# ymxlzgy/commonscenes

Measured on AMD Instinct MI355X. Metric: DDIM denoise steps/sec (32 objects, 16^3 latent), higher is better.
Workload: dtype f32 (operands as fp16 hi+lo pairs, fp32 accumulate)

## Files before the change

### commonscenes_amd/csrc/cs_epilogue.h

```cpp
#pragma once
#include "cs_common.h"

typedef unsigned cs_u32x4 __attribute__((ext_vector_type(4)));

template <class D, class M>
__device__ __forceinline__ f32x4 cs_epi_terms4(const D& d, f32x4 v, M m, int n) {
  if (d.bias) v += *reinterpret_cast<const f32x4*>(d.bias + n);
  if (d.scale) v = v * *reinterpret_cast<const f32x4*>(d.scale + n) + *reinterpret_cast<const f32x4*>(d.shift + n);
  if (d.rowvec) v += *reinterpret_cast<const f32x4*>(d.rowvec + (int64_t)(m / d.rv_rows) * d.ldrv + n);
  if (d.act != CS_ACT_NONE) {
#pragma unroll
    for (int e = 0; e < 4; ++e) v[e] = cs_act(v[e], d.act);
  }
  if (d.res) v += *reinterpret_cast<const f32x4*>(d.res + (int64_t)m * d.ldr + n);
  return v;
}
template <class D>
__device__ __forceinline__ float cs_epi_terms1(const D& d, float v, float bias, float scale, float shift, int m, int n) {
  v += bias;
  if (d.scale) v = v * scale + shift;
  if (d.rowvec) v += d.rowvec[(int64_t)(m / d.rv_rows) * d.ldrv + n];
  v = cs_act(v, d.act);
  if (d.res) v += d.res[(int64_t)m * d.ldr + n];
  return v;
}

__device__ __forceinline__ f32x4 cs_geglu4(f32x4 x, const f32x4& g) {
#pragma unroll
  for (int e = 0; e < 4; ++e) x[e] = x[e] * cs_gelu(g[e]);
  return x;
}

__device__ __forceinline__ cs_u32x4 cs_pair16(const f32x4& v, float out_scale, bool odd, float& oamax) {
  typedef _Float16 h4 __attribute__((ext_vector_type(4)));
  typedef unsigned u32x2 __attribute__((ext_vector_type(2)));
  h4 hi, lo;
#pragma unroll
  for (int e = 0; e < 4; ++e) {
    const float o = v[e] * out_scale;
    oamax = fmaxf(oamax, fabsf(o));
    hi[e] = (_Float16)o;
    lo[e] = (_Float16)(o - (float)hi[e]);
  }
  const u32x2 H = __builtin_bit_cast(u32x2, hi), L = __builtin_bit_cast(u32x2, lo);
  const u32x2 send = odd ? H : L;
  u32x2 recv;
  recv[0] = (unsigned)__builtin_amdgcn_update_dpp(0, (int)send[0], 0xB1, 0xF, 0xF, true);
  recv[1] = (unsigned)__builtin_amdgcn_update_dpp(0, (int)send[1], 0xB1, 0xF, 0xF, true);
  cs_u32x4 r;
  r[0] = odd ? recv[0] : H[0];
  r[1] = odd ? recv[1] : H[1];
  r[2] = odd ? L[0] : recv[0];
  r[3] = odd ? L[1] : recv[1];
  return r;
}
__device__ __forceinline__ cs_u32x4 cs_pair16_half32(const f32x4& v, float out_scale, float& oamax) {
  typedef _Float16 h4 __attribute__((ext_vector_type(4)));
  typedef unsigned u32x2 __attribute__((ext_vector_type(2)));
  h4 hi, lo;
#pragma unroll
  for (int e = 0; e < 4; ++e) {
    const float o = v[e] * out_scale;
    oamax = fmaxf(oamax, fabsf(o));
    hi[e] = (_Float16)o;
    lo[e] = (_Float16)(o - (float)hi[e]);
  }
  const u32x2 H = __builtin_bit_cast(u32x2, hi), L = __builtin_bit_cast(u32x2, lo);
  const auto s0 = __builtin_amdgcn_permlane32_swap(H[0], L[0], false, false);
  const auto s1 = __builtin_amdgcn_permlane32_swap(H[1], L[1], false, false);
  cs_u32x4 r;
  r[0] = s0[0];
  r[1] = s1[0];
  r[2] = s0[1];
  r[3] = s1[1];
  return r;
}
__device__ __forceinline__ int cs_pair_off(int col) { return (col >> 4) * 64 + ((col & 8) ? 32 : 0) + ((col & 4) ? 16 : 0); }
template <class D>
__device__ __forceinline__ void cs_pair_flag(const D& d, bool opair, float oamax) {
  if (opair && d.status && oamax >= 65504.f) atomicOr(d.status, CS_STATUS_F16X3_OVERFLOW);
}

__device__ __forceinline__ void cs_colsum_lanes16(double (*sc)[64], const double (&x)[4], int rl, int cl, double (&tot)[4]) {
  __syncthreads();
#pragma unroll
  for (int e = 0; e < 4; ++e) sc[rl][cl * 4 + e] = x[e];
  __syncthreads();
  if (rl == 0) {
#pragma unroll
    for (int e = 0; e < 4; ++e) {
      double t = 0.0;
      for (int r2 = 0; r2 < 16; ++r2) t += sc[r2][cl * 4 + e];
      tot[e] = t;
    }
  }
}
template <class D>
__device__ __forceinline__ void cs_colsum_staged(const D& d, const float* col, int ld, int rows, int tile, int n) {
  double ts = 0.0, tq = 0.0;
  for (int r2 = 0; r2 < rows; ++r2) {
    const double x = (double)col[r2 * ld];
    ts += x;
    tq += x * x;
  }
  double* o = d.gn_part + ((int64_t)tile * d.gn_ld + n) * 2;
  o[0] = ts;
  o[1] = tq;
}
```

### commonscenes_amd/csrc/cs_gemm_f16x3.hip

```cpp
#include <cstdlib>
#include <cstring>
#include "cs_f16x3.h"
#include "cs_epilogue.h"
#include <type_traits>
#include <utility>

namespace {

using cs16::h8;
using cs16::split8;
using cs16::wait_vmcnt;
using cs16::BKH;
using cs16::A_SCALE_DEFAULT;
using cs16::OOB;
constexpr int MAX_TAPS = 27;
#ifndef CS_ABLATE
#define CS_ABLATE 0
#endif

struct CsClsBatch {
  const void* w[8];
  const void* w_lo[8];
  float acc_scale[8];
  int n;
// ... 51 lines not shown
          f32x4 t[8];
#pragma unroll
          for (int q = 0; q < 8; ++q)
            if (s + q < splits)
              t[q] = __builtin_bit_cast(f32x4, __builtin_amdgcn_raw_buffer_load_b128(wrs, off0 + (unsigned)(s + q) * sstride, 0, 16));
#pragma unroll
          for (int q = 0; q < 8; ++q)
            if (s + q < splits) v += t[q];
        }
        v = cs_epi_terms4(f, v, m, n);
      }
      if (gstat && u < UNITS) *reinterpret_cast<f32x4*>(lv + lrow * BN + 4 * c4) = v;
      if (opair) {
        h4 hi, lo;
#pragma unroll
        for (int e = 0; e < 4; ++e) {
          const float o = v[e] * f.out_scale;
          oamax = fmaxf(oamax, fabsf(o));
          hi[e] = (_Float16)o;
          lo[e] = (_Float16)(o - (float)hi[e]);
        }
        const u32x2 H = __builtin_bit_cast(u32x2, hi), L = __builtin_bit_cast(u32x2, lo);
        const bool odd = tid & 1;
        const u32x2 send = odd ? H : L;
        u32x2 recv;
        recv[0] = (unsigned)__builtin_amdgcn_update_dpp(0, (int)send[0], 0xB1, 0xF, 0xF, true);
        recv[1] = (unsigned)__builtin_amdgcn_update_dpp(0, (int)send[1], 0xB1, 0xF, 0xF, true);
        u32x4 r;
        r[0] = odd ? recv[0] : H[0];
        r[1] = odd ? recv[1] : H[1];
        r[2] = odd ? L[0] : recv[0];
        r[3] = odd ? L[1] : recv[1];
        if (ok) {
          char* row = reinterpret_cast<char*>(f.out + (int64_t)m * f.ldo);
          *reinterpret_cast<u32x4*>(row + (n >> 4) * 64 + ((n & 8) ? 32 : 0) + ((n & 4) ? 16 : 0)) = r;
        }
      } else if (ok) {
        *reinterpret_cast<f32x4*>(f.out + (int64_t)m * f.ldo + n) = v;
      }
    }
    if (gstat) {
      __syncthreads();
      if (tid < BN && n0 + tid < cout) {
        double ts = 0.0, tq = 0.0;
#pragma unroll
        for (int r2 = 0; r2 < 16; ++r2) {
          const double d = (double)lv[r2 * BN + tid];
          ts += d;
          tq += d * d;
        }
        double* o = f.gn_part + ((int64_t)((m0 + r0) / 16) * f.gn_ld + n0 + tid) * 2;
        o[0] = ts;
        o[1] = tq;
      }
      __syncthreads();
    }
  }
  cs_pair_flag(f, opair, oamax);
  __syncthreads();
  if (tid == 0) {
    const int d = __hip_atomic_fetch_add(arrive + 1, 1, __ATOMIC_RELAXED, __HIP_MEMORY_SCOPE_AGENT);
    if (d == R - 1) {
      __hip_atomic_store(arrive, 0, __ATOMIC_RELAXED, __HIP_MEMORY_SCOPE_AGENT);
      __hip_atomic_store(arrive + 1, 0, __ATOMIC_RELAXED, __HIP_MEMORY_SCOPE_AGENT);
    }
  }
}

template <class F, int... I>
__device__ __forceinline__ void static_steps(std::integer_sequence<int, I...>, F&& f) {
  (f(std::integral_constant<int, I>{}), ...);
}

template <int WMB, int WNB, int WAVES_M, int WAVES_N, bool PRE, int SLAB = 0, bool PAIR = false, int TPK = 9, bool PW = false>
__global__ __launch_bounds__(64 * WAVES_M * WAVES_N, 2) void conv_gemm_f16x3_kernel(const CsConvGemm p, int M, int tiles_n,
                                                              int taps_hw, int kw_, int kg_per_tap,
                                                              long long x_bytes, unsigned w_bytes, int vec_epilogue,
                                                              int splits, int omap_f, int omap_p_in, const CsClsBatch cb,
                                                              const CsFuseK fz, int u_base, int u_count) {
  constexpr int BM = 32 * WMB * WAVES_M;
  constexpr int BN = 32 * WNB * WAVES_N;
  constexpr int NW = WAVES_M * WAVES_N;
  constexpr int NT = 64 * NW;
  constexpr bool TR = PW;
  static_assert(!SLAB || (WMB <= 2 && WAVES_N == 1), "slab path: one or two row blocks per wave");
  static_assert(!PAIR || (!PRE && SLAB == 0), "interleaved operand pairs: per-tap gather path only");
  static_assert(TPK == 9 || ((TPK == 4 || TPK == 3) && SLAB != 0), "taps per kd: 3x3 or (slab path only) 2x2 / 3x1");
  static_assert(!PW || SLAB == 0, "pointwise GEMMs take the gather path (there is one tap)");
  constexpr int KW_ = TPK == 9 ? 3 : TPK == 4 ? 2 : 1;
  constexpr int KH_ = TPK / KW_;
  constexpr int SLAB_ROWS = BM + (KH_ - 1) * SLAB + (KW_ - 1);
  constexpr int SLAB_IMG_WI = (SLAB_ROWS + 31) / 32;
  constexpr int SLAB_WI = PRE ? 2 * SLAB_IMG_WI : (SLAB_ROWS + 15) / 16;
  constexpr int SLAB_IMG = SLAB_IMG_WI * 1024;
  constexpr int SLAB_BYTES = SLAB ? SLAB_WI * 1024 : 0;
  constexpr int RING0 = 2 * SLAB_BYTES;
  constexpr int A_BYTES = SLAB ? 0 : BM * 64;
  constexpr int B_BYTES = 2 * BN * 16;
  constexpr int STAGE = A_BYTES + 2 * B_BYTES;
#ifdef CS_RING3
  constexpr int NSTAGE = 3;
#else
#ifdef CS_PW_RING3
  constexpr int NSTAGE = (BM == 64 && BN == 64) ? 6 : (TPK == 4 ? 4 : 3);
#else
#ifndef CS_RING64
#define CS_RING64 6
#endif
  constexpr int NSTAGE = (BM == 64 && BN == 64) ? CS_RING64 : ((TPK == 4 || (PW && BM == 256 && BN == 224)) ? 4 : 3);
#endif
#endif
  constexpr int PF = NSTAGE - 1;
  constexpr int DUMP = RING0 + NSTAGE * STAGE;
  constexpr int ROWBASE = DUMP + 1024;
  constexpr int DELTA = ROWBASE + (SLAB ? 0 : BM * 4);
  constexpr int ROWMIN = DELTA + (SLAB ? 0 : MAX_TAPS * BM * 2);
  constexpr int EP_KU = (4 * (32 * WNB / 4) + 63) / 64;
  constexpr int EPI_NEED = NW * (16 * 32 * WNB) + NW * 2 * EP_KU * 1024 + 2048;
  constexpr int OTAB = ((ROWMIN + 16 > EPI_NEED) ? ROWMIN + 16 : EPI_NEED);
  constexpr int LDS_BYTES = OTAB + (TPK == 4 ? BM * 4 : 0);
  constexpr short INVALID = (short)0x8000;
  constexpr int A_WI = BM / 16;
  constexpr int B_WI = BN / 32;
  constexpr int A_PW = SLAB ? 0 : A_WI / NW;
  constexpr int A_PWN = A_PW > 0 ? A_PW : 1;
  constexpr int B_PW = (2 * B_WI + NW - 1) / NW;
  constexpr int D = A_PW + B_PW;
  static_assert(A_WI % NW == 0, "A tile must split evenly over the waves");
  static_assert(D <= 7, "vmcnt immediates");
  __shared__ __attribute__((aligned(16))) unsigned char smem[LDS_BYTES];

  const int tid = threadIdx.x;
  const int lane = tid & 63;
  const int wave = __builtin_amdgcn_readfirstlane(tid >> 6);
  const int l31 = lane & 31;
  const int half = lane >> 5;
  const int wm0 = (wave / WAVES_N) * (32 * WMB);
  const int wn0 = (wave % WAVES_N) * (32 * WNB);

  int tile;
  {
    const int nblk = gridDim.x, b = blockIdx.x;
    const int q = nblk >> 3, r = nblk & 7, xcd = b & 7, within = b >> 3;
    tile = (xcd < r ? xcd * (q + 1) : r * (q + 1) + (xcd - r) * q) + within;
  }
  const void* w_hi_ = p.w;
  const void* w_lo_ = p.w_lo;
  float acc_scale_ = p.acc_scale;
  int pad_d = p.pd, pad_h = p.ph, pad_w = p.pw, omap_p = omap_p_in;
  int cls_id = 0;
  if constexpr (TPK == 4) {
    if (cb.n > 1) {
      const int per_cls = ((M + BM - 1) / BM) * tiles_n * splits;
      const int cls = tile / per_cls;
      cls_id = cls;
      tile -= cls * per_cls;
      w_hi_ = cb.w[cls];
      w_lo_ = cb.w_lo[cls];
      acc_scale_ = cb.acc_scale[cls];
      const int nw = 1 + (omap_f & 1), nh = 1 + ((omap_f >> 1) & 1);
      const int qw = cls % nw, qh = (cls / nw) % nh, qd = cls / (nw * nh);
      pad_d = (omap_f & 4) ? 1 - qd : 1;
      pad_h = (omap_f & 2) ? 1 - qh : 1;
      pad_w = (omap_f & 1) ? 1 - qw : 1;
      omap_p = (qd << 2) | (qh << 1) | qw;
    }
  }
// ... 113 lines not shown
  const int nk = 0;
#else
  const int nk = max(0, min(nk_all, k_first + per_split) - k_first);
#endif

  int a_rowbase[A_PWN];
  unsigned a_piece[A_PWN];
  int a_rowidx[A_PWN];
#pragma unroll
  for (int i = 0; i < A_PW; ++i) {
    const int w = wave * A_PW + i;
    if constexpr (PRE) {
      const int within = w % (A_WI / 2);
      const int row = 32 * within + (lane >> 1);
      a_rowidx[i] = row;
      if constexpr (PW) a_rowbase[i] = (m0 + row < M) ? row : -1;
      else a_rowbase[i] = rowbase[row] - row_lo;
      a_piece[i] = (unsigned)(((lane & 1) ^ ((row >> 3) & 1)) * 8);
    } else {
      const int row = 16 * w + (lane >> 2);
      a_rowidx[i] = row;
      if constexpr (PW) a_rowbase[i] = (m0 + row < M) ? row : -1;
      else a_rowbase[i] = rowbase[row] - row_lo;
      a_piece[i] = (unsigned)(((lane & 3) ^ ((row >> 2) & 3)) * 4);
    }
  }
  unsigned b_off[B_PW];
#pragma unroll
  for (int i = 0; i < B_PW; ++i) {
    const int v = wave * B_PW + i;
    const int img = v / B_WI;
    const int u = (v - img * B_WI) * 64 + lane;
    const int kg = u / BN;
    const int n = u - kg * BN;
    b_off[i] = (v < 2 * B_WI && n0 + n < p.cout) ? (unsigned)((kg * p.cout + n0 + n) * 16) : OOB;
  }

  auto issue_dma = [&](int tap, int cc, int stage) {
    unsigned char* st = smem + RING0 + stage * STAGE;
    const bool skip_a = ((CS_ABLATE & 128) && tap % 3 != 0) || ((CS_ABLATE & 256) && tap % 9 != 0);
#pragma unroll
    for (int i = 0; i < A_PW; ++i) {
      if (skip_a) break;
      const int c = cc * BKH + (int)a_piece[i];
      constexpr unsigned ESZ = PRE ? 2u : 4u;
      unsigned off;
      if constexpr (PW) {
        off = (a_rowbase[i] >= 0 && c < p.cin) ? (unsigned)a_rowbase[i] * ((unsigned)p.lda * ESZ) + (unsigned)c * ESZ : OOB;
      } else {
        const short dl = delta[tap * BM + a_rowidx[i]];
        off = (dl != INVALID && c < p.cin)
                  ? (unsigned)(a_rowbase[i] + (int)dl) * ((unsigned)p.lda * ESZ) + (unsigned)c * ESZ
                  : OOB;
      }
      if (CS_ABLATE & 2) off = OOB;
      if ((CS_ABLATE & 64) && off != OOB) off &= 0x3FF0u;
      const int w = wave * A_PW + i;
      if constexpr (PRE) {
        if (w >= A_WI / 2)
          __builtin_amdgcn_raw_ptr_buffer_load_lds(xlrs, st + w * 1024, 16, off, 0, 0, 0);
        else
          __builtin_amdgcn_raw_ptr_buffer_load_lds(xrs, st + w * 1024, 16, off, 0, 0, 0);
      } else {
        __builtin_amdgcn_raw_ptr_buffer_load_lds(xrs, st + w * 1024, 16, off, 0, 0, 0);
      }
    }
    const unsigned kbase = (unsigned)((tap * kg_per_tap + cc * 2) * p.cout) * 16u;
#pragma unroll
    for (int i = 0; i < B_PW; ++i) {
      const int v = wave * B_PW + i;
      const int img = v / B_WI;
      unsigned off = (b_off[i] == OOB || cc >= chunks_per_tap) ? OOB : b_off[i] + kbase;
      if (CS_ABLATE & 2) off = OOB;
      if ((CS_ABLATE & 64) && off != OOB) off &= 0x3FF0u;
      unsigned char* dst = (v < 2 * B_WI) ? st + A_BYTES + img * B_BYTES + (v - img * B_WI) * 1024 : smem + DUMP;
      if (img == 1)
        __builtin_amdgcn_raw_ptr_buffer_load_lds(lrs, dst, 16, off, 0, 0, 0);
      else
        __builtin_amdgcn_raw_ptr_buffer_load_lds(hrs, dst, 16, off, 0, 0, 0);
    }
  };

  constexpr int TRV = ROWBASE;
  if constexpr (TR) {
    static_assert(TRV + 2048 <= LDS_BYTES && BN <= 256 && (BN + 63) / 64 <= NW, "bias / row-vector rows beyond the ring");
    if (wave < (BN + 63) / 64) {
      const unsigned col = (unsigned)(64 * wave + lane);
      const unsigned off = col < (unsigned)BN ? (unsigned)(n0 + (int)col) * 4u : OOB;
      float* const tv = reinterpret_cast<float*>(smem + TRV);
      if (p.bias) {
        const __amdgpu_buffer_rsrc_t brs = __builtin_amdgcn_make_buffer_rsrc((void*)p.bias, 0, (unsigned)p.cout * 4u, 0x00020000);
        __builtin_amdgcn_raw_ptr_buffer_load_lds(brs, tv + 64 * wave, 4, off, 0, 0, 0);
      }
      if (p.rowvec) {
        const __amdgpu_buffer_rsrc_t vrs = __builtin_amdgcn_make_buffer_rsrc(
            (void*)(p.rowvec + (int64_t)(m0 / p.rv_rows) * p.ldrv), 0, (unsigned)p.cout * 4u, 0x00020000);
        __builtin_amdgcn_raw_ptr_buffer_load_lds(vrs, tv + 256 + 64 * wave, 4, off, 0, 0, 0);
      }
    }
  }

  f32x16 acc[WMB][WNB];
#pragma unroll
  for (int i = 0; i < WMB; ++i)
#pragma unroll
    for (int j = 0; j < WNB; ++j)
#pragma unroll
      for (int r = 0; r < 16; ++r) acc[i][j][r] = 0.f;

  int dtap = k_first % ntaps, dcc = k_first / ntaps;
  auto advance = [&]() {
    if (++dtap == ntaps) {
      dtap = 0;
      ++dcc;
    }
  };
#pragma unroll
  for (int q = 0; q < PF; ++q) {
    issue_dma(dtap, dcc, q);
    advance();
  }

  int a_frag[WMB][2];
#pragma unroll
  for (int i = 0; i < WMB; ++i) {
    const int row = wm0 + 32 * i + l31;
    if constexpr (PRE) {
      a_frag[i][0] = row * 32 + ((half ^ ((row >> 3) & 1)) * 16);
      a_frag[i][1] = a_frag[i][0] + BM * 32;
    } else {
      const int s = (row >> 2) & 3;
      a_frag[i][0] = row * 64 + (((2 * half) ^ s) * 16);
      a_frag[i][1] = row * 64 + (((2 * half + 1) ^ s) * 16);
    }
  }
  const int b_frag = A_BYTES + (half * BN + wn0 + l31) * 16;

  float amax = 0.f;
  auto load_a = [&](int st, h8 (&hi)[WMB], h8 (&lo)[WMB]) {
    const unsigned char* s = smem + RING0 + st * STAGE;
#pragma unroll
    for (int i = 0; i < WMB; ++i) {
      if constexpr (PRE) {
        hi[i] = *reinterpret_cast<const h8*>(s + a_frag[i][0]);
        lo[i] = *reinterpret_cast<const h8*>(s + a_frag[i][1]);
      } else {
        const f32x4 x0 = *reinterpret_cast<const f32x4*>(s + a_frag[i][0]);
        const f32x4 x1 = *reinterpret_cast<const f32x4*>(s + a_frag[i][1]);
#if CS_ABLATE & 512
        hi[i] = __builtin_bit_cast(h8, x0);
        lo[i] = __builtin_bit_cast(h8, x1);
#else
        if constexpr (PAIR) {
          hi[i] = __builtin_bit_cast(h8, x0);
          lo[i] = __builtin_bit_cast(h8, x1);
        } else {
          split8(x0, x1, a_scale, hi[i], lo[i], amax);
        }
#endif
      }
    }
  };
  constexpr int SLAB_PW = (SLAB_WI + NW - 1) / NW;
  const int s_w = p.win, s_hw = p.hin * p.win;
  const int s_rows = p.nb * p.din * s_hw;
  const int s_need = BM + (KH_ - 1) * s_w + (KW_ - 1);
  unsigned vmask[WMB];
// ... 84 lines not shown
    hi = __builtin_bit_cast(h8, x0);
    lo = __builtin_bit_cast(h8, x1);
    (void)m9;
#else
    cs16::split8_masked(x0, x1, ((m9 >> t9) & 1u) ? a_scale : 0.f, hi, lo, amax);
#endif
  };

  h8 ah[WMB], al[WMB];
  if constexpr (SLAB != 0) {
    const int sc0 = k_first / TPK;
    issue_slab(sc0);
    wait_vmcnt<0>();
    __builtin_amdgcn_s_barrier();
#pragma unroll
    for (int i = 0; i < WMB; ++i)
      load_a_slab(std::integral_constant<int, 0>{}, i, sc0 & 1, (vmask[i] >> (TPK * (sc0 % KD))) & ((1u << TPK) - 1u), ah[i],
                  al[i]);
  } else {
  wait_vmcnt<(PF - 1) * D>();
  __builtin_amdgcn_s_barrier();
  load_a(0, ah, al);
  }

  auto step = [&](auto stage_c) {
    constexpr int stage = decltype(stage_c)::value;
    constexpr int nstage = (stage + 1) % NSTAGE;
    constexpr int dstage = (stage + PF) % NSTAGE;
    if (!(CS_ABLATE & 4)) wait_vmcnt<(PF - 2) * D + B_PW>();
    if (!(CS_ABLATE & 8)) __builtin_amdgcn_s_barrier();
    const unsigned char* s = smem + RING0 + stage * STAGE;
    h8 ah2[WMB], al2[WMB];
#if CS_ABLATE & 16
    __builtin_amdgcn_s_setprio(1);
#endif
#pragma unroll
    for (int j = 0; j < WNB; ++j) {
      const h8 bh = *reinterpret_cast<const h8*>(s + b_frag + j * 512);
      const h8 bl = *reinterpret_cast<const h8*>(s + b_frag + B_BYTES + j * 512);
#pragma unroll
      for (int i = 0; i < WMB; ++i) {
        if constexpr (TR) {
          acc[i][j] = __builtin_amdgcn_mfma_f32_32x32x16_f16(bh, al[i], acc[i][j], 0, 0, 0);
          acc[i][j] = __builtin_amdgcn_mfma_f32_32x32x16_f16(bl, ah[i], acc[i][j], 0, 0, 0);
          acc[i][j] = __builtin_amdgcn_mfma_f32_32x32x16_f16(bh, ah[i], acc[i][j], 0, 0, 0);
        } else {
          acc[i][j] = __builtin_amdgcn_mfma_f32_32x32x16_f16(al[i], bh, acc[i][j], 0, 0, 0);
          acc[i][j] = __builtin_amdgcn_mfma_f32_32x32x16_f16(ah[i], bl, acc[i][j], 0, 0, 0);
          acc[i][j] = __builtin_amdgcn_mfma_f32_32x32x16_f16(ah[i], bh, acc[i][j], 0, 0, 0);
        }
      }
      if (j == 0) {
        if (!(CS_ABLATE & 1)) issue_dma(dtap, dcc, dstage);
        advance();
        load_a(nstage, ah2, al2);
      }
    }
#if CS_ABLATE & 16
    __builtin_amdgcn_s_setprio(0);
#endif
#pragma unroll
    for (int i = 0; i < WMB; ++i) {
      ah[i] = ah2[i];
      al[i] = al2[i];
    }
  };
  auto sstep = [&](auto stage_c, auto t9_c, int sc, const unsigned (&m9_this)[WMB], const unsigned (&m9_next)[WMB]) {
    constexpr int stage = decltype(stage_c)::value;
    constexpr int t9 = decltype(t9_c)::value;
    constexpr int dstage = (stage + PF) % NSTAGE;
    if (!(CS_ABLATE & 4)) wait_vmcnt<((t9 >= 1 && t9 <= PF - 1) ? SLAB_PW : 0) + (PF - 1) * B_PW>();
    if (!(CS_ABLATE & 8)) __builtin_amdgcn_s_barrier();
    const unsigned char* s = smem + RING0 + stage * STAGE;
    h8 ah2[WMB], al2[WMB];
    h8 bh, bl;
#pragma unroll
    for (int j = 0; j < WNB; ++j) {
      if (!(((CS_ABLATE & 4096) && (j & 1)) || ((CS_ABLATE & 8192) && j > 0))) {
        bh = *reinterpret_cast<const h8*>(s + b_frag + j * 512);
        bl = *reinterpret_cast<const h8*>(s + b_frag + B_BYTES + j * 512);
      }
#pragma unroll
      for (int i = 0; i < WMB; ++i) {
        acc[i][j] = __builtin_amdgcn_mfma_f32_32x32x16_f16(al[i], bh, acc[i][j], 0, 0, 0);
        acc[i][j] = __builtin_amdgcn_mfma_f32_32x32x16_f16(ah[i], bl, acc[i][j], 0, 0, 0);
        acc[i][j] = __builtin_amdgcn_mfma_f32_32x32x16_f16(ah[i], bh, acc[i][j], 0, 0, 0);
      }
      if (j == 0) {
        if constexpr (t9 == 0) issue_slab(sc + 1);
        issue_dma(dtap, dcc, dstage);
        advance();
#pragma unroll
        for (int i = 0; i < WMB; ++i) {
          if constexpr (t9 == TPK - 1)
            load_a_slab(std::integral_constant<int, 0>{}, i, (sc + 1) & 1, m9_next[i], ah2[i], al2[i]);
          else
            load_a_slab(std::integral_constant<int, t9 + 1>{}, i, sc & 1, m9_this[i], ah2[i], al2[i]);
        }
      }
    }
#pragma unroll
    for (int i = 0; i < WMB; ++i) {
      ah[i] = ah2[i];
      al[i] = al2[i];
    }
  };
  if constexpr (SLAB != 0) {
    static_assert(((TPK == 9 || TPK == 3) && NSTAGE == 3) || (TPK == 4 && NSTAGE == 4), "a chunk's ring stage is its tap index mod NSTAGE");
    const int sc_first = k_first / TPK, sc_end = sc_first + nk / TPK;
    int kdc = sc_first % KD;
    constexpr unsigned TMASK = (1u << TPK) - 1u;
    for (int sc = sc_first; sc < sc_end; ++sc) {
      const int kdn = kdc == KD - 1 ? 0 : kdc + 1;
      unsigned m9[WMB], m9n[WMB];
#pragma unroll
      for (int i = 0; i < WMB; ++i) {
        m9[i] = (vmask[i] >> (TPK * kdc)) & TMASK;
        m9n[i] = (vmask[i] >> (TPK * kdn)) & TMASK;
      }
      if constexpr (TPK == 9) {
        sstep(std::integral_constant<int, 0>{}, std::integral_constant<int, 0>{}, sc, m9, m9n);
        sstep(std::integral_constant<int, 1>{}, std::integral_constant<int, 1>{}, sc, m9, m9n);
        sstep(std::integral_constant<int, 2>{}, std::integral_constant<int, 2>{}, sc, m9, m9n);
        sstep(std::integral_constant<int, 0>{}, std::integral_constant<int, 3>{}, sc, m9, m9n);
        sstep(std::integral_constant<int, 1>{}, std::integral_constant<int, 4>{}, sc, m9, m9n);
        sstep(std::integral_constant<int, 2>{}, std::integral_constant<int, 5>{}, sc, m9, m9n);
        sstep(std::integral_constant<int, 0>{}, std::integral_constant<int, 6>{}, sc, m9, m9n);
        sstep(std::integral_constant<int, 1>{}, std::integral_constant<int, 7>{}, sc, m9, m9n);
        sstep(std::integral_constant<int, 2>{}, std::integral_constant<int, 8>{}, sc, m9, m9n);
      } else if constexpr (TPK == 3) {
        sstep(std::integral_constant<int, 0>{}, std::integral_constant<int, 0>{}, sc, m9, m9n);
        sstep(std::integral_constant<int, 1>{}, std::integral_constant<int, 1>{}, sc, m9, m9n);
        sstep(std::integral_constant<int, 2>{}, std::integral_constant<int, 2>{}, sc, m9, m9n);
      } else {
        sstep(std::integral_constant<int, 0>{}, std::integral_constant<int, 0>{}, sc, m9, m9n);
        sstep(std::integral_constant<int, 1>{}, std::integral_constant<int, 1>{}, sc, m9, m9n);
        sstep(std::integral_constant<int, 2>{}, std::integral_constant<int, 2>{}, sc, m9, m9n);
        sstep(std::integral_constant<int, 3>{}, std::integral_constant<int, 3>{}, sc, m9, m9n);
      }
      kdc = kdn;
    }
  } else
  for (int kc = 0; kc < nk; kc += NSTAGE) {
    step(std::integral_constant<int, 0>{});
    static_steps(std::make_integer_sequence<int, NSTAGE - 1>{}, [&](auto s1) {
      constexpr int st = decltype(s1)::value + 1;
      if (kc + st < nk) step(std::integral_constant<int, st>{});
    });
  }
  wait_vmcnt<0>();
  if constexpr (!PRE && !PAIR) {
    if (p.status && amax >= 65504.f) atomicOr(p.status, CS_STATUS_F16X3_OVERFLOW);
  }

#if CS_ABLATE & 1024
  {
    float sum = 0.f;
#pragma unroll
    for (int i = 0; i < WMB; ++i)
#pragma unroll
      for (int j = 0; j < WNB; ++j)
#pragma unroll
        for (int r = 0; r < 16; ++r) sum += acc[i][j][r];
    if (M == -12345) p.out[tid] = sum;
    return;
  }
#endif
  float* const outp = p.out + ((int64_t)cls_id * splits + split) * M * p.ldo;
  const bool omap = (TPK == 4) && (omap_f & 7) != 0 && !(omap_f & 8);
  int* const otab = reinterpret_cast<int*>(smem + OTAB);
  long long ob = m0, Mo = M;
  int ospan = BM;
  if constexpr (TPK == 4) {
    if (omap) {
      const int fd = 1 + ((omap_f >> 2) & 1), fh = 1 + ((omap_f >> 1) & 1), fw = 1 + (omap_f & 1);
      const int qd = (omap_p >> 2) & 1, qh = (omap_p >> 1) & 1, qw = omap_p & 1;
      auto orow = [&](int m) -> long long {
        const int w = m % p.win;
        int t = m / p.win;
        const int h = t % p.hin;
        t /= p.hin;
        const int d = t % p.din;
        const int n = t / p.din;
        return (((long long)n * (p.din * fd) + d * fd + qd) * (p.hin * fh) + h * fh + qh) * (p.win * fw) + w * fw + qw;
      };
      ob = orow(m0);
      Mo = (long long)M * (fd * fh * fw);
      const int mlast = min(m0 + BM, M) - 1;
      ospan = (int)(orow(mlast) - ob) + 1;
      for (int r = tid; r < BM; r += NT) otab[r] = (m0 + r < M) ? (int)(orow(m0 + r) - ob) : 0;
      __syncthreads();
    }
  }
  auto orel = [&](int row) -> int { return omap ? otab[row] : row; };
  constexpr int WCOLS = 32 * WNB;
  constexpr int PASS_R = (NW * 16 * WCOLS * 4 <= DUMP) ? 8 : 4;
  constexpr int EPI_ROWS = 2 * PASS_R;
  constexpr int EPI_BYTES = EPI_ROWS * WCOLS * 4;
  static_assert(NW * EPI_BYTES <= DUMP, "epilogue staging must fit in the ring");
  {
    typedef cs_u32x4 u32x4;
    constexpr int QR = 2;
    constexpr int NQ = 16 / QR;
    constexpr int UPR = WCOLS / 4;
    constexpr int UN = 2 * QR * UPR;
    constexpr int KU = (UN + 63) / 64;
    constexpr int EPB = 2 * QR * WCOLS * 4;
    constexpr int RSLAB = KU * 1024;
    constexpr int RES0 = NW * EPB;
    constexpr int VEC0 = RES0 + NW * 2 * RSLAB;
    constexpr int BNV = (BN + 63) / 64;
    static_assert(VEC0 + 2048 <= LDS_BYTES && BN <= 256 && BNV <= NW, "pipelined epilogue must fit in the kernel's LDS");
    const int m_last = min(m0 + BM, M) - 1;
    const bool geglu = p.act == CS_ACT_GEGLU;
    const bool has_res = p.res != nullptr;
#ifndef CS_PIPED_PLAIN
#define CS_PIPED_PLAIN 1
#endif
    const bool piped = !(CS_ABLATE & 32) && vec_epilogue && (p.res || p.bias || p.rowvec || CS_PIPED_PLAIN) && !p.scale && splits == 1 &&
                       (!geglu || n0 + BN <= p.cout) && (!p.rowvec || (m0 / p.rv_rows == m_last / p.rv_rows)) &&
                       (long long)ospan * p.ldo * 4 < 0x7FF00000LL && (!p.res || (long long)BM * p.ldr * 4 < 0x7FF00000LL);
    const bool gstat = p.gn_part != nullptr;
    const bool opair = p.out_format == 2;
    if ((gstat || opair) && !piped && tid == 0 && p.status) atomicOr(p.status, CS_STATUS_INTERNAL);
    if constexpr (TR) {
      if (piped && !gstat) {
        typedef cs_u32x4 u32x4;
        constexpr int NG = 4 * WNB;
        constexpr int GB = (WMB * NG <= 16) ? NG : NG / 2;
        static_assert(NG % GB == 0 && WMB * GB <= 16, "residual batches");
        const long long o_skip = (long long)m0 * p.ldo * 4, r_skip = (long long)m0 * p.ldr * 4;
        const long long o_cols = geglu ? p.cout / 2 : p.cout;
        const long long o_left = ((long long)(M - 1) * p.ldo + o_cols) * 4 - o_skip;
        const long long r_left = has_res ? ((long long)(M - 1) * p.ldr + p.cout) * 4 - r_skip : 0;
        const __amdgpu_buffer_rsrc_t ors = __builtin_amdgcn_make_buffer_rsrc(
            (void*)((char*)p.out + o_skip), 0, o_left > 0x7FF00000LL ? 0x7FF00000u : (unsigned)o_left, 0x00020000);
        const __amdgpu_buffer_rsrc_t rrs = __builtin_amdgcn_make_buffer_rsrc(
            (void*)(has_res ? (const char*)p.res + r_skip : (const char*)p.out), 0,
            r_left > 0x7FF00000LL ? 0x7FF00000u : (r_left > 0 ? (unsigned)r_left : 0u), 0x00020000);
        const float* const tvb = reinterpret_cast<const float*>(smem + TRV) + wn0 + 4 * half;
        const float* const tvr = tvb + 256;
        const int cl = n0 + wn0 + 4 * half;
        bool rok[WMB];
        unsigned orow[WMB], rrow[WMB];
#pragma unroll
        for (int i = 0; i < WMB; ++i) {
          const int row = wm0 + 32 * i + l31;
          rok[i] = m0 + row < M;
          orow[i] = (unsigned)(row * p.ldo) * 4u;
          rrow[i] = (unsigned)(row * p.ldr) * 4u;
        }
        float oamax = 0.f;
        if (geglu) {
          constexpr int HG = NG / 2;
          const int co = (n0 + wn0) / 2 + 4 * half;
#pragma unroll
          for (int t = 0; t < HG; ++t) {
            f32x4 bx = {0.f, 0.f, 0.f, 0.f}, bg = bx;
            if (p.bias) {
              bx = *reinterpret_cast<const f32x4*>(tvb + 8 * t);
              bg = *reinterpret_cast<const f32x4*>(tvb + 8 * (t + HG));
            }
#pragma unroll
            for (int i = 0; i < WMB; ++i) {
              f32x4 xv, gv;
#pragma unroll
              for (int e = 0; e < 4; ++e) {
                xv[e] = acc[i][t / 4][4 * (t % 4) + e] * acc_scale_;
                gv[e] = acc[i][(t + HG) / 4][4 * ((t + HG) % 4) + e] * acc_scale_;
              }
              if (p.bias) {
                xv += bx;
                gv += bg;
              }
              xv = (CS_ABLATE & 32768) ? xv * gv : cs_geglu4(xv, gv);
              const bool ok = rok[i];
              if (opair) {
                if (!ok) xv = f32x4{0.f, 0.f, 0.f, 0.f};
                const u32x4 pk = cs_pair16_half32(xv, p.out_scale, oamax);
                unsigned off = ok ? orow[i] + (unsigned)cs_pair_off(co + 8 * t) : OOB;
                if (CS_ABLATE & 16384) off = OOB;
                __builtin_amdgcn_raw_buffer_store_b128(pk, ors, off, 0, 0);
              } else {
                unsigned off = ok ? orow[i] + (unsigned)(co + 8 * t) * 4u : OOB;
                if (CS_ABLATE & 16384) off = OOB;
                __builtin_amdgcn_raw_buffer_store_b128(__builtin_bit_cast(u32x4, xv), ors, off, 0, 0);
              }
            }
          }
        } else {
#pragma unroll
          for (int t0 = 0; t0 < NG; t0 += GB) {
            f32x4 rv[WMB][GB];
            if (has_res) {
#pragma unroll
              for (int i = 0; i < WMB; ++i)
#pragma unroll
                for (int tt = 0; tt < GB; ++tt) {
                  const int n = cl + 8 * (t0 + tt);
                  const unsigned off = (rok[i] && n < p.cout) ? rrow[i] + (unsigned)n * 4u : OOB;
                  rv[i][tt] = __builtin_bit_cast(f32x4, __builtin_amdgcn_raw_buffer_load_b128(rrs, off, 0, 0));
                }
            }
#pragma unroll
            for (int tt = 0; tt < GB; ++tt) {
              const int t = t0 + tt;
              const int n = cl + 8 * t;
              f32x4 bv = {0.f, 0.f, 0.f, 0.f}, vv = bv;
              if (p.bias) bv = *reinterpret_cast<const f32x4*>(tvb + 8 * t);
              if (p.rowvec) vv = *reinterpret_cast<const f32x4*>(tvr + 8 * t);
#pragma unroll
              for (int i = 0; i < WMB; ++i) {
                f32x4 v;
#pragma unroll
                for (int e = 0; e < 4; ++e) v[e] = acc[i][t / 4][4 * (t % 4) + e] * acc_scale_;
                if (p.bias) v += bv;
                if (p.rowvec) v += vv;
                if (p.act != CS_ACT_NONE) {
#pragma unroll
                  for (int e = 0; e < 4; ++e) v[e] = cs_act(v[e], p.act);
                }
                if (has_res) v += rv[i][tt];
                const bool ok = rok[i] && n < p.cout;
                if (opair) {
                  if (!ok) v = f32x4{0.f, 0.f, 0.f, 0.f};
                  const u32x4 pk = cs_pair16_half32(v, p.out_scale, oamax);
                  unsigned off = ok ? orow[i] + (unsigned)cs_pair_off(n) : OOB;
                  if (CS_ABLATE & 16384) off = OOB;
                  __builtin_amdgcn_raw_buffer_store_b128(pk, ors, off, 0, 0);
                } else {
                  unsigned off = ok ? orow[i] + (unsigned)n * 4u : OOB;
                  if (CS_ABLATE & 16384) off = OOB;
                  __builtin_amdgcn_raw_buffer_store_b128(__builtin_bit_cast(u32x4, v), ors, off, 0, 0);
                }
              }
            }
          }
        }
        cs_pair_flag(p, opair, oamax);
        return;
      }
      {
        static_assert(NW * 32 * 33 * 4 <= DUMP, "untranspose scratch must fit in the ring");
        __syncthreads();
        float* const tb = reinterpret_cast<float*>(smem) + wave * (32 * 33);
#pragma unroll
        for (int i = 0; i < WMB; ++i)
#pragma unroll
          for (int j = 0; j < WNB; ++j) {
#pragma unroll
            for (int r = 0; r < 16; ++r) tb[l31 * 33 + 8 * (r >> 2) + 4 * half + (r & 3)] = acc[i][j][r];
#pragma unroll
            for (int r = 0; r < 16; ++r) acc[i][j][r] = tb[(8 * (r >> 2) + 4 * half + (r & 3)) * 33 + l31];
          }
      }
    }
    if (piped) {
      __syncthreads();
      float* const ep = reinterpret_cast<float*>(smem + wave * EPB);
      typedef float f32x2 __attribute__((ext_vector_type(2)));
      f32x2 gs[KU][2], gq[KU][2];
#pragma unroll
      for (int k = 0; k < KU; ++k)
#pragma unroll
        for (int e = 0; e < 2; ++e) gs[k][e] = gq[k][e] = f32x2{0.f, 0.f};
      float oamax = 0.f;
      float* const rs = reinterpret_cast<float*>(smem + RES0 + wave * 2 * RSLAB);
      float* const vb = reinterpret_cast<float*>(smem + VEC0);
      float* const vr = vb + 256;
      const long long o_skip = ob * p.ldo * 4, r_skip = (long long)m0 * p.ldr * 4;
      const long long o_left = ((Mo - 1) * p.ldo + p.cout) * 4 - o_skip;
      const long long r_left = has_res ? ((long long)(M - 1) * p.ldr + p.cout) * 4 - r_skip : 0;
      const long long o_cols = geglu ? p.cout / 2 : p.cout;
      const long long o_left2 = ((Mo - 1) * p.ldo + o_cols) * 4 - o_skip;
      (void)o_left;
      const __amdgpu_buffer_rsrc_t ors = __builtin_amdgcn_make_buffer_rsrc(
          (void*)((char*)p.out + o_skip), 0, o_left2 > 0x7FF00000LL ? 0x7FF00000u : (unsigned)o_left2, 0x00020000);
      const __amdgpu_buffer_rsrc_t rrs = __builtin_amdgcn_make_buffer_rsrc(
          (void*)(has_res ? (const char*)p.res + r_skip : (const char*)p.out), 0,
          r_left > 0x7FF00000LL ? 0x7FF00000u : (r_left > 0 ? (unsigned)r_left : 0u), 0x00020000);
      if (wave < BNV) {
        const unsigned col = (unsigned)(64 * wave + lane);
        const unsigned off = col < (unsigned)BN ? (unsigned)(n0 + (int)col) * 4u : OOB;
        if (p.bias) {
          const __amdgpu_buffer_rsrc_t brs = __builtin_amdgcn_make_buffer_rsrc((void*)p.bias, 0, (unsigned)p.cout * 4u, 0x00020000);
          __builtin_amdgcn_raw_ptr_buffer_load_lds(brs, vb + 64 * wave, 4, off, 0, 0, 0);
        }
        if (p.rowvec) {
          const __amdgpu_buffer_rsrc_t vrs = __builtin_amdgcn_make_buffer_rsrc(
              (void*)(p.rowvec + (int64_t)(m0 / p.rv_rows) * p.ldrv), 0, (unsigned)p.cout * 4u, 0x00020000);
          __builtin_amdgcn_raw_ptr_buffer_load_lds(vrs, vr + 64 * wave, 4, off, 0, 0, 0);
        }
      }
      auto pass_row = [&](int i, int q, int lrow) {
        return wm0 + 32 * i + 2 * (q & 1) + 8 * (q >> 1) + (lrow & 1) + 4 * (lrow >> 1);
      };
      auto fetch_res = [&](int pass) {
        const int i = pass / NQ, q = pass - i * NQ;
#pragma unroll
        for (int k = 0; k < KU; ++k) {
          const int u = lane + 64 * k;
          const int lrow = u / UPR, c4 = u - lrow * UPR;
          const int row = pass_row(i, q, lrow & 3);
          const unsigned off = (u < UN && m0 + row < M) ? (unsigned)(row * p.ldr + n0 + wn0 + 4 * c4) * 4u : OOB;
          __builtin_amdgcn_raw_ptr_buffer_load_lds(rrs, rs + (pass & 1) * (RSLAB / 4) + 256 * k, 16, off, 0, 0, 0);
        }
      };
      if (has_res) {
        fetch_res(0);
        wait_vmcnt<KU>();
      } else {
        wait_vmcnt<0>();
      }
      __syncthreads();
      constexpr int NPASS = WMB * NQ;
      auto do_pass = [&](auto i_c, auto q_c) {
        constexpr int i = decltype(i_c)::value, q = decltype(q_c)::value, pass = i * NQ + q;
        if (has_res) {
          if constexpr (pass + 1 < NPASS) fetch_res(pass + 1);
          wait_vmcnt<(pass > 0 ? KU : 0) + (pass + 1 < NPASS ? KU : 0)>();
        }
#pragma unroll
        for (int j = 0; j < WNB; ++j)
// ... 450 lines not shown
```

Before: 16.18.

## Store transposed MFMA accumulators as row lines via quad DPP transpose

Adds a 4x4 quad transpose via DPP so each lane holds four consecutive output columns of one row, and applies it in two places. It writes 128-bit row-contiguous stores for the pointwise GEMM epilogue (selected tile shapes) and for the 3x1-tap slab conv path, which now computes with swapped MFMA operands (transposed accumulator). The aim is to replace scattered or LDS-untransposed stores with coalesced line stores and to skip the LDS untranspose scratch for bare 3x1 convs. The cost is extra DPP shuffles, more register pressure, and more template variants.

After: 16.66, median of 6. 2.9% higher.

```diff
diff --git a/commonscenes_amd/csrc/cs_epilogue.h b/commonscenes_amd/csrc/cs_epilogue.h
--- a/commonscenes_amd/csrc/cs_epilogue.h
+++ b/commonscenes_amd/csrc/cs_epilogue.h
@@ -75,6 +75,29 @@
   r[3] = s1[1];
   return r;
 }
+__device__ __forceinline__ void cs_quad_transpose4(f32x4 (&x)[4], int lane) {
+  const bool o1 = lane & 1, o2 = lane & 2;
+#pragma unroll
+  for (int s = 0; s < 4; s += 2)
+#pragma unroll
+    for (int e = 0; e < 4; ++e) {
+      const float a = x[s][e], b = x[s + 1][e];
+      const float recv = __builtin_bit_cast(
+          float, __builtin_amdgcn_update_dpp(0, __builtin_bit_cast(int, o1 ? a : b), 0xB1, 0xF, 0xF, true));
+      x[s][e] = o1 ? recv : a;
+      x[s + 1][e] = o1 ? b : recv;
+    }
+#pragma unroll
+  for (int s = 0; s < 2; ++s)
+#pragma unroll
+    for (int e = 0; e < 4; ++e) {
+      const float a = x[s][e], b = x[s + 2][e];
+      const float recv = __builtin_bit_cast(
+          float, __builtin_amdgcn_update_dpp(0, __builtin_bit_cast(int, o2 ? a : b), 0x4E, 0xF, 0xF, true));
+      x[s][e] = o2 ? recv : a;
+      x[s + 2][e] = o2 ? b : recv;
+    }
+}
 __device__ __forceinline__ int cs_pair_off(int col) { return (col >> 4) * 64 + ((col & 8) ? 32 : 0) + ((col & 4) ? 16 : 0); }
 template <class D>
 __device__ __forceinline__ void cs_pair_flag(const D& d, bool opair, float oamax) {
diff --git a/commonscenes_amd/csrc/cs_gemm_f16x3.hip b/commonscenes_amd/csrc/cs_gemm_f16x3.hip
--- a/commonscenes_amd/csrc/cs_gemm_f16x3.hip
+++ b/commonscenes_amd/csrc/cs_gemm_f16x3.hip
@@ -157,7 +157,14 @@
   constexpr int BN = 32 * WNB * WAVES_N;
   constexpr int NW = WAVES_M * WAVES_N;
   constexpr int NT = 64 * NW;
-  constexpr bool TR = PW;
+#ifndef CS_LINE_POS
+#define CS_LINE_POS 1
+#endif
+#ifndef CS_LINE_PW
+#define CS_LINE_PW 1
+#endif
+  constexpr bool TR = PW || (TPK == 3 && CS_LINE_POS);
+  constexpr bool LINE = TPK == 3 || CS_LINE_PW == 2 || (CS_LINE_PW == 1 && BM == 256 && BN == 224);
   static_assert(!SLAB || (WMB <= 2 && WAVES_N == 1), "slab path: one or two row blocks per wave");
   static_assert(!PAIR || (!PRE && SLAB == 0), "interleaved operand pairs: per-tap gather path only");
   static_assert(TPK == 9 || ((TPK == 4 || TPK == 3) && SLAB != 0), "taps per kd: 3x3 or (slab path only) 2x2 / 3x1");
@@ -437,7 +444,7 @@
   };
 
   constexpr int TRV = ROWBASE;
-  if constexpr (TR) {
+  if constexpr (PW) {
     static_assert(TRV + 2048 <= LDS_BYTES && BN <= 256 && (BN + 63) / 64 <= NW, "bias / row-vector rows beyond the ring");
     if (wave < (BN + 63) / 64) {
       const unsigned col = (unsigned)(64 * wave + lane);
@@ -688,9 +695,15 @@
       }
 #pragma unroll
       for (int i = 0; i < WMB; ++i) {
-        acc[i][j] = __builtin_amdgcn_mfma_f32_32x32x16_f16(al[i], bh, acc[i][j], 0, 0, 0);
-        acc[i][j] = __builtin_amdgcn_mfma_f32_32x32x16_f16(ah[i], bl, acc[i][j], 0, 0, 0);
-        acc[i][j] = __builtin_amdgcn_mfma_f32_32x32x16_f16(ah[i], bh, acc[i][j], 0, 0, 0);
+        if constexpr (TR) {
+          acc[i][j] = __builtin_amdgcn_mfma_f32_32x32x16_f16(bh, al[i], acc[i][j], 0, 0, 0);
+          acc[i][j] = __builtin_amdgcn_mfma_f32_32x32x16_f16(bl, ah[i], acc[i][j], 0, 0, 0);
+          acc[i][j] = __builtin_amdgcn_mfma_f32_32x32x16_f16(bh, ah[i], acc[i][j], 0, 0, 0);
+        } else {
+          acc[i][j] = __builtin_amdgcn_mfma_f32_32x32x16_f16(al[i], bh, acc[i][j], 0, 0, 0);
+          acc[i][j] = __builtin_amdgcn_mfma_f32_32x32x16_f16(ah[i], bl, acc[i][j], 0, 0, 0);
+          acc[i][j] = __builtin_amdgcn_mfma_f32_32x32x16_f16(ah[i], bh, acc[i][j], 0, 0, 0);
+        }
       }
       if (j == 0) {
         if constexpr (t9 == 0) issue_slab(sc + 1);
@@ -830,6 +843,190 @@
     const bool opair = p.out_format == 2;
     if ((gstat || opair) && !piped && tid == 0 && p.status) atomicOr(p.status, CS_STATUS_INTERNAL);
     if constexpr (TR) {
+      const int q4 = l31 & 3, r4 = l31 & ~3;
+      if constexpr (TPK == 3) {
+        const bool bare = !p.bias && !p.scale && !p.rowvec && !p.res && p.act == CS_ACT_NONE && !gstat && !opair;
+        if (!(CS_ABLATE & 32) && vec_epilogue && bare && (long long)BM * p.ldo * 4 < 0x7FF00000LL) {
+          typedef cs_u32x4 u32x4;
+          const int rows = min(BM, M - m0);
+          const __amdgpu_buffer_rsrc_t ors = __builtin_amdgcn_make_buffer_rsrc(
+              (void*)(outp + (int64_t)m0 * p.ldo), 0, (unsigned)(((int64_t)(rows - 1) * p.ldo + p.cout) * 4), 0x00020000);
+          const int cq = n0 + wn0 + 8 * q4 + 4 * half;
+#pragma unroll
+          for (int i = 0; i < WMB; ++i) {
+            const int row0 = wm0 + 32 * i + r4;
+            const unsigned orow = (unsigned)(row0 * p.ldo) * 4u;
+#pragma unroll
+            for (int j = 0; j < WNB; ++j) {
+              f32x4 v[4];
+#pragma unroll
+              for (int g = 0; g < 4; ++g)
+#pragma unroll
+                for (int e = 0; e < 4; ++e) v[g][e] = acc[i][j][4 * g + e] * acc_scale_;
+              cs_quad_transpose4(v, lane);
+              const int n = cq + 32 * j;
+#pragma unroll
+              for (int s = 0; s < 4; ++s) {
+                unsigned off = (row0 + s < rows && n < p.cout) ? orow + (unsigned)(s * p.ldo + n) * 4u : OOB;
+                if (CS_ABLATE & 16384) off = OOB;
+                __builtin_amdgcn_raw_buffer_store_b128(__builtin_bit_cast(u32x4, v[s]), ors, off, 0, 0);
+              }
+            }
+          }
+          return;
+        }
+      }
+      if constexpr (PW && LINE) {
+      if (piped && !gstat) {
+        typedef cs_u32x4 u32x4;
+        constexpr int JB = (4 * WMB * WNB <= 16) ? WNB : 4 / WMB;
+        static_assert(JB >= 1 && 4 * WMB * JB <= 16, "residual batches");
+        const long long o_skip = (long long)m0 * p.ldo * 4, r_skip = (long long)m0 * p.ldr * 4;
+        const long long o_cols = geglu ? p.cout / 2 : p.cout;
+        const long long o_left = ((long long)(M - 1) * p.ldo + o_cols) * 4 - o_skip;
+        const long long r_left = has_res ? ((long long)(M - 1) * p.ldr + p.cout) * 4 - r_skip : 0;
+        const __amdgpu_buffer_rsrc_t ors = __builtin_amdgcn_make_buffer_rsrc(
+            (void*)((char*)p.out + o_skip), 0, o_left > 0x7FF00000LL ? 0x7FF00000u : (unsigned)o_left, 0x00020000);
+        const __amdgpu_buffer_rsrc_t rrs = __builtin_amdgcn_make_buffer_rsrc(
+            (void*)(has_res ? (const char*)p.res + r_skip : (const char*)p.out), 0,
+            r_left > 0x7FF00000LL ? 0x7FF00000u : (r_left > 0 ? (unsigned)r_left : 0u), 0x00020000);
+        const float* const tvb = reinterpret_cast<const float*>(smem + TRV) + wn0 + 4 * half;
+        const float* const tvr = tvb + 256;
+        int nrow[WMB];
+        unsigned orow[WMB], rrow[WMB];
+#pragma unroll
+        for (int i = 0; i < WMB; ++i) {
+          const int row0 = wm0 + 32 * i + r4;
+          nrow[i] = M - m0 - row0;
+          orow[i] = (unsigned)(row0 * p.ldo) * 4u;
+          rrow[i] = (unsigned)(row0 * p.ldr) * 4u;
+        }
+        const unsigned ostep = (unsigned)p.ldo * 4u, rstep = (unsigned)p.ldr * 4u;
+        float oamax = 0.f;
+        if (geglu) {
+          constexpr int HG = 2 * WNB;
+          const int co = (n0 + wn0) / 2 + 8 * q4 + 4 * half;
+#pragma unroll
+          for (int b = 0; b < (HG + 3) / 4; ++b) {
+            f32x4 bx[4], bg[4];
+#pragma unroll
+            for (int g = 0; g < 4; ++g) {
+              bx[g] = bg[g] = f32x4{0.f, 0.f, 0.f, 0.f};
+              if (4 * b + g < HG && p.bias) {
+                bx[g] = *reinterpret_cast<const f32x4*>(tvb + 8 * (4 * b + g));
+                bg[g] = *reinterpret_cast<const f32x4*>(tvb + 8 * (4 * b + g + HG));
+              }
+            }
+            const bool cok = 4 * b + q4 < HG;
+#pragma unroll
+            for (int i = 0; i < WMB; ++i) {
+              f32x4 v[4];
+#pragma unroll
+              for (int g = 0; g < 4; ++g) {
+                v[g] = f32x4{0.f, 0.f, 0.f, 0.f};
+                const int t = 4 * b + g;
+                if (t < HG) {
+                  f32x4 xv, gv;
+#pragma unroll
+                  for (int e = 0; e < 4; ++e) {
+                    xv[e] = acc[i][t / 4][4 * (t % 4) + e] * acc_scale_;
+                    gv[e] = acc[i][(t + HG) / 4][4 * ((t + HG) % 4) + e] * acc_scale_;
+                  }
+                  if (p.bias) {
+                    xv += bx[g];
+                    gv += bg[g];
+                  }
+                  v[g] = (CS_ABLATE & 32768) ? xv * gv : cs_geglu4(xv, gv);
+                }
+              }
+              cs_quad_transpose4(v, lane);
+#pragma unroll
+              for (int s = 0; s < 4; ++s) {
+                const bool ok = cok && s < nrow[i];
+                if (opair) {
+                  if (!ok) v[s] = f32x4{0.f, 0.f, 0.f, 0.f};
+                  const u32x4 pk = cs_pair16_half32(v[s], p.out_scale, oamax);
+                  unsigned off = ok ? orow[i] + (unsigned)s * ostep + (unsigned)cs_pair_off(co + 32 * b) : OOB;
+                  if (CS_ABLATE & 16384) off = OOB;
+                  __builtin_amdgcn_raw_buffer_store_b128(pk, ors, off, 0, 0);
+                } else {
+                  unsigned off = ok ? orow[i] + (unsigned)s * ostep + (unsigned)(co + 32 * b) * 4u : OOB;
+                  if (CS_ABLATE & 16384) off = OOB;
+                  __builtin_amdgcn_raw_buffer_store_b128(__builtin_bit_cast(u32x4, v[s]), ors, off, 0, 0);
+                }
+              }
+            }
+          }
+        } else {
+          const int cq = n0 + wn0 + 8 * q4 + 4 * half;
+#pragma unroll
+          for (int j0 = 0; j0 < WNB; j0 += JB) {
+            f32x4 rv[WMB][JB][4];
+            if (has_res) {
+#pragma unroll
+              for (int i = 0; i < WMB; ++i)
+#pragma unroll
+                for (int jj = 0; jj < JB; ++jj)
+#pragma unroll
+                  for (int s = 0; s < 4; ++s) {
+                    if (j0 + jj >= WNB) continue;
+                    const int n = cq + 32 * (j0 + jj);
+                    const unsigned off = (s < nrow[i] && n < p.cout) ? rrow[i] + (unsigned)s * rstep + (unsigned)n * 4u : OOB;
+                    rv[i][jj][s] = __builtin_bit_cast(f32x4, __builtin_amdgcn_raw_buffer_load_b128(rrs, off, 0, 0));
+                  }
+            }
+#pragma unroll
+            for (int jj = 0; jj < JB; ++jj) {
+              const int j = j0 + jj;
+              if (j >= WNB) continue;
+              f32x4 bv[4], vv[4];
+#pragma unroll
+              for (int g = 0; g < 4; ++g) {
+                bv[g] = vv[g] = f32x4{0.f, 0.f, 0.f, 0.f};
+                if (p.bias) bv[g] = *reinterpret_cast<const f32x4*>(tvb + 32 * j + 8 * g);
+                if (p.rowvec) vv[g] = *reinterpret_cast<const f32x4*>(tvr + 32 * j + 8 * g);
+              }
+              const int n = cq + 32 * j;
+#pragma unroll
+              for (int i = 0; i < WMB; ++i) {
+                f32x4 v[4];
+#pragma unroll
+                for (int g = 0; g < 4; ++g) {
+#pragma unroll
+                  for (int e = 0; e < 4; ++e) v[g][e] = acc[i][j][4 * g + e] * acc_scale_;
+                  if (p.bias) v[g] += bv[g];
+                  if (p.rowvec) v[g] += vv[g];
+                  if (p.act != CS_ACT_NONE) {
+#pragma unroll
+                    for (int e = 0; e < 4; ++e) v[g][e] = cs_act(v[g][e], p.act);
+                  }
+                }
+                cs_quad_transpose4(v, lane);
+#pragma unroll
+                for (int s = 0; s < 4; ++s) {
+                  if (has_res) v[s] += rv[i][jj][s];
+                  const bool ok = s < nrow[i] && n < p.cout;
+                  if (opair) {
+                    if (!ok) v[s] = f32x4{0.f, 0.f, 0.f, 0.f};
+                    const u32x4 pk = cs_pair16_half32(v[s], p.out_scale, oamax);
+                    unsigned off = ok ? orow[i] + (unsigned)s * ostep + (unsigned)cs_pair_off(n) : OOB;
+                    if (CS_ABLATE & 16384) off = OOB;
+                    __builtin_amdgcn_raw_buffer_store_b128(pk, ors, off, 0, 0);
+                  } else {
+                    unsigned off = ok ? orow[i] + (unsigned)s * ostep + (unsigned)n * 4u : OOB;
+                    if (CS_ABLATE & 16384) off = OOB;
+                    __builtin_amdgcn_raw_buffer_store_b128(__builtin_bit_cast(u32x4, v[s]), ors, off, 0, 0);
+                  }
+                }
+              }
+            }
+          }
+        }
+        cs_pair_flag(p, opair, oamax);
+        return;
+      }
+      }
+      if constexpr (PW && !LINE) {
       if (piped && !gstat) {
         typedef cs_u32x4 u32x4;
         constexpr int NG = 4 * WNB;
@@ -945,6 +1142,7 @@
         }
         cs_pair_flag(p, opair, oamax);
         return;
+      }
       }
       {
         static_assert(NW * 32 * 33 * 4 <= DUMP, "untranspose scratch must fit in the ring");
```
